# danieleschmidt/Graph-Hypernetwork-Forge

Measured on AMD Instinct MI355X. Metric: edges/s (HyperGNN forward), higher is better.
Workload: dtype f32; 1 GPU; synthetic uniform KG 1M nodes / 10M edges / 64 rel, hidden 128, L=3 (BASELINE config 3); nodes=1000000, edges=10000000, relations=64, hidden_dim=128, layers=3, text_dim=64, plan=cached (warm), launch=one C-ABI call per kernel, parallelism=single GPU

## Files before the change

### graph-hypernetwork-forge_amd/csrc/weightgen.hip

```cpp
#include "common.h"

namespace ghf {

constexpr int WG_MAX_WIDTH = 1024;
constexpr int WG_UNROLL = 8;
constexpr int WG_HU = 8;

struct HeadPtrs {
    const float* w[3][8];
    const float* b[3][8];
};
constexpr int WG_MAX_L = 8;
struct HeadPtrsL { HeadPtrs p[WG_MAX_L]; };

__global__ __launch_bounds__(256) void wg_hidden_kernel(const float* __restrict__ text_emb, HeadPtrsL PL,
                                                        int R, int T, int Hh, int num_hidden,
                                                        float* __restrict__ hidden_ws, float* __restrict__ acts,
                                                        const float* __restrict__ drop ) {
    __shared__ float buf[2][WG_MAX_WIDTH];
    const int r = blockIdx.x, head = blockIdx.y;
    const HeadPtrs& P = PL.p[blockIdx.z];
    if (hidden_ws) hidden_ws += (size_t)blockIdx.z * 3 * R * (num_hidden ? Hh : T);
    for (int k = threadIdx.x; k < T; k += blockDim.x) buf[0][k] = text_emb[(size_t)r * T + k];
    __syncthreads();
    int cur = 0, in_dim = T;
    const int lane = threadIdx.x & 63, wv = threadIdx.x >> 6, nw = blockDim.x >> 6;
    for (int li = 0; li < num_hidden; ++li) {
        const float* __restrict__ W = P.w[head][li];
        const float* __restrict__ B = P.b[head][li];
        for (int j0 = wv * WG_HU; j0 < Hh; j0 += nw * WG_HU) {
            float s[WG_HU];
#pragma unroll
            for (int u = 0; u < WG_HU; ++u) s[u] = 0.f;
            for (int k = lane; k < in_dim; k += 64) {
                const float xk = buf[cur][k];
#pragma unroll
                for (int u = 0; u < WG_HU; ++u)
                    if (j0 + u < Hh) s[u] = fmaf(xk, W[(size_t)(j0 + u) * in_dim + k], s[u]);
            }
#pragma unroll
            for (int u = 0; u < WG_HU; ++u) {
                const float t = wave_sum(s[u]);
                if (lane == 0 && j0 + u < Hh) {
                    const float a = fmaxf(t + B[j0 + u], 0.f);
                    buf[cur ^ 1][j0 + u] = drop ? a * drop[(((size_t)head * num_hidden + li) * R + r) * Hh + j0 + u] : a;
                }
            }
        }
        __syncthreads();
        cur ^= 1;
        in_dim = Hh;
        if (acts) {
            float* a = acts + (((size_t)head * num_hidden + li) * R + r) * Hh;
            for (int k = threadIdx.x; k < Hh; k += blockDim.x) a[k] = buf[cur][k];
        }
    }
    if (!hidden_ws) return;
    float* out = hidden_ws + ((size_t)head * R + r) * in_dim;
    for (int k = threadIdx.x; k < in_dim; k += blockDim.x) out[k] = buf[cur][k];
}

__device__ __forceinline__ size_t frag16_index(int r, int kk, int o, int d) {
    const int NT = d >> 4, NJ2 = d >> 3;
    return ((((size_t)r * NT + (o >> 4)) * NJ2 + (kk >> 4)) * 64 + (((kk & 15) >> 2) << 4) + (o & 15)) * 4 + (kk & 3);
}

__global__ __launch_bounds__(256) void wg_out_simple_kernel(const float* __restrict__ z ,
                                                            const float* __restrict__ W3, const float* __restrict__ b3,
                                                            const float* __restrict__ log_scale,
                                                            int R, int Hl, int n_out, int head, int d_in, int d_out,
                                                            int layout, size_t rstride, float* __restrict__ out) {
    const int lane = threadIdx.x & 63;
    const int n = blockIdx.x * 4 + (threadIdx.x >> 6);
    if (n >= n_out) return;
    const float scale = expf(log_scale[0]);
    const float bn = b3[n];
    for (int r0 = 0; r0 < R; r0 += WG_UNROLL) {
      float sv[WG_UNROLL];
#pragma unroll
      for (int u = 0; u < WG_UNROLL; ++u) sv[u] = 0.f;
      for (int k = lane; k < Hl; k += 64) {
          const float wk = W3[(size_t)n * Hl + k];
#pragma unroll
          for (int u = 0; u < WG_UNROLL; ++u)
              if (r0 + u < R) sv[u] = fmaf(z[(size_t)(r0 + u) * Hl + k], wk, sv[u]);
      }
#pragma unroll
      for (int u = 0; u < WG_UNROLL; ++u) {
        const int r = r0 + u;
        const float s = wave_sum(sv[u]);
        if (lane == 0 && r < R) {
            const float v = (s + bn) * scale;
            if (head == 2 || layout == GHF_WLAYOUT_NATURAL) {
                out[(size_t)r * rstride + n] = v;
            } else {
                const int i = n / d_out, o = n - i * d_out;
                out[frag16_index(r, head * d_in + i, o, d_out)] = v;
            }
        }
      }
    }
}

typedef float f32x4 __attribute__((ext_vector_type(4)));

template <int LAYOUT>
__global__ __launch_bounds__(256) void wg_out_mfma_kernel(const float* __restrict__ z ,
                                                          const float* __restrict__ W3, const float* __restrict__ b3,
                                                          const float* __restrict__ log_scale,
                                                          int R, int Hl, int n_out, int head, int d, size_t rstride,
                                                          float* __restrict__ out) {
    const int lane = threadIdx.x & 63, wv = threadIdx.x >> 6;
    const int q = lane >> 4, c16 = lane & 15;
    const int mt = blockIdx.x * 4 + wv;
    if (mt * 16 >= n_out) return;
    int n_a;
    int o = 0, it = 0;
    if (LAYOUT != GHF_WLAYOUT_NATURAL) {
        const int tiles_per_o = d >> 4;
        o = mt / tiles_per_o;
        it = mt - o * tiles_per_o;
        n_a = (16 * it + c16) * d + o;
    } else {
        n_a = 16 * mt + c16;
    }
    const bool a_ok = n_a < n_out;
    const float* __restrict__ arow = W3 + (size_t)(a_ok ? n_a : 0) * Hl + 4 * q;
    const float scale = expf(log_scale[0]);
    const int NJ = Hl >> 4;

    for (int r0 = 0; r0 < R; r0 += 16) {
        const int rc = r0 + c16;
        const bool b_ok = rc < R;
        const float* __restrict__ brow = z + (size_t)(b_ok ? rc : 0) * Hl + 4 * q;
        f32x4 acc = {0.f, 0.f, 0.f, 0.f};
        for (int j = 0; j < NJ; ++j) {
            f32x4 a = *(const f32x4*)(arow + 16 * j);
            f32x4 b = *(const f32x4*)(brow + 16 * j);
            if (!a_ok) a = (f32x4){0.f, 0.f, 0.f, 0.f};
            if (!b_ok) b = (f32x4){0.f, 0.f, 0.f, 0.f};
#pragma unroll
            for (int s = 0; s < 4; ++s) acc = __builtin_amdgcn_mfma_f32_16x16x4f32(a[s], b[s], acc, 0, 0, 0);
        }
        if (!b_ok) continue;
        if (LAYOUT == GHF_WLAYOUT_FRAG16) {
            f32x4 v;
#pragma unroll
            for (int s = 0; s < 4; ++s) {
                const int n = (16 * it + 4 * q + s) * d + o;
                v[s] = (acc[s] + b3[n]) * scale;
            }
            const int kk0 = head * d + 16 * it + 4 * q;
            *(f32x4*)(out + frag16_index(rc, kk0, o, d)) = v;
        } else {
#pragma unroll
            for (int s = 0; s < 4; ++s) {
                const int n = 16 * mt + 4 * q + s;
                if (n < n_out) out[(size_t)rc * rstride + n] = (acc[s] + b3[n]) * scale;
            }
        }
    }
}

struct OutHeads {
    const float* z[3];
    const float* W3[3];
    const float* b3[3];
    const float* log_scale[3];
    float* out[3];
    int n_out[3];
    size_t rstride[3];
};
struct OutHeadsL { OutHeads h[WG_MAX_L]; };
template <int NJT>
__global__ __launch_bounds__(256) void wg_out_mfma3_kernel(OutHeadsL HL, int R, int Hl) {
    const int head = blockIdx.y % 3;
    const OutHeads& H = HL.h[blockIdx.y / 3];
    const float* __restrict__ z = H.z[head];
    const float* __restrict__ W3 = H.W3[head];
    const float* __restrict__ b3 = H.b3[head];
    float* __restrict__ out = H.out[head];
    const int n_out = H.n_out[head];
    const size_t rstride = H.rstride[head];
    const int lane = threadIdx.x & 63, wv = threadIdx.x >> 6;
    const int q = lane >> 4, c16 = lane & 15;
    const int mt = blockIdx.x * 4 + wv;
    if (mt * 16 >= n_out) return;
    const int n_a = 16 * mt + c16;
    const bool a_ok = n_a < n_out;
    const float* __restrict__ arow = W3 + (size_t)(a_ok ? n_a : 0) * Hl + 4 * q;
    const float scale = expf(H.log_scale[head][0]);
    const int NJ = Hl >> 4;
    if constexpr (NJT > 0) {
        f32x4 a[NJT];
#pragma unroll
        for (int j = 0; j < NJT; ++j) {
            a[j] = *(const f32x4*)(arow + 16 * j);
            if (!a_ok) a[j] = (f32x4){0.f, 0.f, 0.f, 0.f};
        }
        for (int r0 = 0; r0 < R; r0 += 16) {
            const int rc = r0 + c16;
            const bool b_ok = rc < R;
            const float* __restrict__ brow = z + (size_t)(b_ok ? rc : 0) * Hl + 4 * q;
            f32x4 b[NJT];
#pragma unroll
            for (int j = 0; j < NJT; ++j) {
                b[j] = *(const f32x4*)(brow + 16 * j);
                if (!b_ok) b[j] = (f32x4){0.f, 0.f, 0.f, 0.f};
            }
            f32x4 acc = {0.f, 0.f, 0.f, 0.f};
#pragma unroll
            for (int j = 0; j < NJT; ++j)
#pragma unroll
                for (int s = 0; s < 4; ++s) acc = __builtin_amdgcn_mfma_f32_16x16x4f32(a[j][s], b[j][s], acc, 0, 0, 0);
            if (!b_ok) continue;
#pragma unroll
            for (int s = 0; s < 4; ++s) {
                const int n = 16 * mt + 4 * q + s;
                if (n < n_out) out[(size_t)rc * rstride + n] = (acc[s] + b3[n]) * scale;
            }
        }
        return;
    }
    for (int r0 = 0; r0 < R; r0 += 16) {
        const int rc = r0 + c16;
        const bool b_ok = rc < R;
        const float* __restrict__ brow = z + (size_t)(b_ok ? rc : 0) * Hl + 4 * q;
        f32x4 acc = {0.f, 0.f, 0.f, 0.f};
        for (int j = 0; j < NJ; ++j) {
            f32x4 a = *(const f32x4*)(arow + 16 * j);
            f32x4 b = *(const f32x4*)(brow + 16 * j);
            if (!a_ok) a = (f32x4){0.f, 0.f, 0.f, 0.f};
            if (!b_ok) b = (f32x4){0.f, 0.f, 0.f, 0.f};
#pragma unroll
            for (int s = 0; s < 4; ++s) acc = __builtin_amdgcn_mfma_f32_16x16x4f32(a[s], b[s], acc, 0, 0, 0);
        }
        if (!b_ok) continue;
#pragma unroll
        for (int s = 0; s < 4; ++s) {
            const int n = 16 * mt + 4 * q + s;
            if (n < n_out) out[(size_t)rc * rstride + n] = (acc[s] + b3[n]) * scale;
        }
    }
}

struct PackL { float* W[WG_MAX_L]; };
__global__ __launch_bounds__(1024) void wg_pack2h_kernel(PackL WL, int R, int d, int32_t* __restrict__ range_flag) {
    float* __restrict__ W = WL.W[blockIdx.y];
    float* __restrict__ scales = W + (size_t)R * 2 * d * d;
    extern __shared__ float wbuf[];
    __shared__ float red[16];
    __shared__ int cnt[2];
    __shared__ WeakRows weak_red[16];
    if (threadIdx.x < 2) cnt[threadIdx.x] = 0;
    const int r = blockIdx.x, tid = threadIdx.x, n = 2 * d * d;
    float* __restrict__ mine = W + (size_t)r * n;
    float mx = 0.f;
    for (int i = tid; i < n / 4; i += 1024) {
        const float4 v = ((const float4*)mine)[i];
        ((float4*)wbuf)[i] = v;
        mx = fmaxf(fmaxf(mx, fmaxf(fabsf(v.x), fabsf(v.y))), fmaxf(fabsf(v.z), fabsf(v.w)));
    }
    mx = wave_absmax(mx);
    if ((tid & 63) == 0) red[tid >> 6] = mx;
    __syncthreads();
    mx = 0.f;
    for (int i = 0; i < 16; ++i) mx = fmaxf(mx, red[i]);
    {
        WeakRows wr;
        wr.init();
        const int lane = tid & 63, wv = tid >> 6;
        for (int row = wv; row < 2 * d; row += 16) {
            float s = 0.f;
            for (int o = lane; o < d; o += 64) s += fabsf(wbuf[row * d + o]);
            wr.add(row >= d, wave_sum(s));
        }
        if (lane == 0) weak_red[wv] = wr;
    }
    const int sh = split2h_shift(mx);
    const float up = pow2f(sh);
    if (tid == 0) scales[r] = pow2f(-sh);
    const int NKS = d >> 4;
    _Float16* __restrict__ dst = (_Float16*)mine;
    for (int g = tid; g < n / 8; g += 1024) {
        const int slot = g & 63, fk = g >> 6;
        const int ks = fk % NKS, ct = fk / NKS;
        const int o = ct * 16 + (slot & 15), kk0 = ks * 32 + (slot >> 4) * 8;
        _Float16 hi[8], lo[8];
        int tiny = 0, nz = 0;
#pragma unroll
        for (int e = 0; e < 8; ++e) {
            const float xs = wbuf[(kk0 + e) * d + o] * up;
            split2h(xs, hi[e], lo[e]);
            tiny += range_tiny(xs);
            nz += xs != 0.f;
        }
        _Float16* p = dst + ((size_t)fk * 2 * 64 + slot) * 8;
#pragma unroll
        for (int e = 0; e < 8; ++e) { p[e] = hi[e]; p[512 + e] = lo[e]; }
        if (tiny) atomicAdd(&cnt[0], tiny);
        if (nz) atomicAdd(&cnt[1], nz);
    }
    __syncthreads();
    if (tid == 0) {
        range_raise(range_flag, GHF_RANGE_WEIGHTS, cnt[0], cnt[1]);
        WeakRows wr = weak_red[0];
        for (int i = 1; i < 16; ++i) wr.merge(weak_red[i]);
        range_raise_weak(range_flag, wr, d);
    }
}

int launch_weightgen_acts(const float* text_emb, const float* const* head_params, int R, int T, int Hh, int num_hidden,
                          float* acts, const float* hidden_drop, hipStream_t stream) {
    GHF_REQUIRE(R > 0 && T > 0 && num_hidden >= 0 && num_hidden <= 7, "weightgen_acts: bad shape");
    GHF_REQUIRE(T <= WG_MAX_WIDTH && Hh <= WG_MAX_WIDTH, "weightgen_acts: text_dim/hidden_dim > %d unsupported", WG_MAX_WIDTH);
    if (num_hidden == 0) return GHF_OK;
    HeadPtrsL PL;
    HeadPtrs& P = PL.p[0];
    const int nl = num_hidden + 1;
    for (int h = 0; h < 3; ++h)
        for (int l = 0; l < nl; ++l) {
            P.w[h][l] = head_params[(h * nl + l) * 2 + 0];
            P.b[h][l] = head_params[(h * nl + l) * 2 + 1];
        }
    wg_hidden_kernel<<<dim3(R, 3, 1), 256, 0, stream>>>(text_emb, PL, R, T, Hh, num_hidden, nullptr, acts, hidden_drop);
    GHF_LAUNCH_CHECK();
    return GHF_OK;
}

__global__ __launch_bounds__(256) void wg_combine_kernel(const float* __restrict__ top, const float* __restrict__ bottom,
                                                         int transpose, int d, float* __restrict__ out) {
    const int r = blockIdx.y;
    const int n = 2 * d * d;
    for (int idx = blockIdx.x * 256 + threadIdx.x; idx < n; idx += gridDim.x * 256) {
        const int kk = idx / d, o = idx - kk * d;
        const float* src = kk < d ? top : bottom;
        const int k = kk < d ? kk : kk - d;
        float v = 0.f;
        if (src) v = transpose ? src[((size_t)r * d + o) * d + k] : src[((size_t)r * d + k) * d + o];
        out[(size_t)r * n + idx] = v;
    }
}

__global__ __launch_bounds__(256) void wg_combine_frag16_kernel(const float* __restrict__ top, const float* __restrict__ bottom,
                                                                int transpose, int d, float* __restrict__ out) {
    const int r = blockIdx.y;
    const int n = 2 * d * d;
    for (int idx = blockIdx.x * 256 + threadIdx.x; idx < n; idx += gridDim.x * 256) {
        const int kk = idx / d, o = idx - kk * d;
        const float* src = kk < d ? top : bottom;
        const int k = kk < d ? kk : kk - d;
        float v = 0.f;
        if (src) v = transpose ? src[((size_t)r * d + o) * d + k] : src[((size_t)r * d + k) * d + o];
        out[frag16_index(r, kk, o, d)] = v;
    }
}

int launch_weights_pack(const float* top, const float* bottom, int transpose, int R, int d, int layout, float* out,
                        hipStream_t stream) {
    GHF_REQUIRE(R > 0 && d > 0 && out, "weights_pack: bad arguments");
    if (layout == GHF_WLAYOUT_FRAG16) {
        GHF_REQUIRE((d % 16) == 0, "weights_pack: FRAG16 needs d %% 16 == 0");
        wg_combine_frag16_kernel<<<dim3(32, (unsigned)R), 256, 0, stream>>>(top, bottom, transpose, d, out);
        GHF_LAUNCH_CHECK();
        return GHF_OK;
    }
    GHF_REQUIRE(layout == GHF_WLAYOUT_SPLIT2H, "weights_pack: layout %d is not packed from natural matrices here", layout);
    GHF_REQUIRE((d % 32) == 0 && (size_t)2 * d * d * 4 <= 128 * 1024, "weights_pack: SPLIT2H needs d %% 32 == 0, d <= 128");
    wg_combine_kernel<<<dim3(32, (unsigned)R), 256, 0, stream>>>(top, bottom, transpose, d, out);
    GHF_LAUNCH_CHECK();
    const size_t lds = (size_t)2 * d * d * 4;
    GHF_SET_MAX_LDS(wg_pack2h_kernel, lds);
    PackL WL;
    WL.W[0] = out;
    wg_pack2h_kernel<<<dim3(R, 1), 1024, lds, stream>>>(WL, R, d, range_flag_ptr());
    GHF_LAUNCH_CHECK();
    return GHF_OK;
}

int launch_weightgen_batched(int L, const float* text_emb, const float* const* head_params, const float* const* log_scales,
                             int R, int T, int Hh, int num_hidden, int d_in, int d_out, int layout,
                             float* hidden_ws, float* const* W_msg, float* const* W_self, float* const* bias,
                             const float* hidden_drop, hipStream_t stream, float* acts) {
    GHF_REQUIRE(L >= 1 && L <= WG_MAX_L, "weightgen: %d generators per call (1..%d)", L, WG_MAX_L);
    GHF_REQUIRE(R > 0 && T > 0 && d_in > 0 && d_out > 0, "weightgen: R, T, d_in, d_out must be positive");
    GHF_REQUIRE(num_hidden >= 0 && num_hidden <= 7, "weightgen: num_hidden=%d outside [0,7]", num_hidden);
    GHF_REQUIRE(num_hidden == 0 || Hh > 0, "weightgen: hidden_dim must be positive");
    GHF_REQUIRE(T <= WG_MAX_WIDTH && Hh <= WG_MAX_WIDTH, "weightgen: text_dim/hidden_dim > %d unsupported", WG_MAX_WIDTH);
    GHF_REQUIRE(layout == GHF_WLAYOUT_NATURAL || layout == GHF_WLAYOUT_FRAG16 || layout == GHF_WLAYOUT_SPLIT2H, "weightgen: bad layout %d", layout);
    GHF_REQUIRE((!hidden_drop && !acts) || L == 1, "weightgen: dropout masks / saved activations go with one generator per call");
    for (int g = 0; g < L; ++g) {
        GHF_REQUIRE(W_msg[g] && bias[g], "weightgen: null output pointer (generator %d)", g);
        if (layout == GHF_WLAYOUT_SPLIT2H)
            GHF_REQUIRE(d_in == d_out && (d_in % 32) == 0 && (size_t)2 * d_in * d_out * 4 <= 128 * 1024 && (!W_self || W_self[g] == nullptr),
                        "weightgen: SPLIT2H needs d_in == d_out, d %% 32 == 0, d <= 128 and W_self == NULL");
        if (layout == GHF_WLAYOUT_FRAG16)
            GHF_REQUIRE(d_in == d_out && (d_in % 16) == 0 && (!W_self || W_self[g] == nullptr),
                        "weightgen: FRAG16 needs d_in == d_out, d %% 16 == 0 and W_self == NULL");
        else if (layout == GHF_WLAYOUT_NATURAL)
            GHF_REQUIRE(W_self && W_self[g] != nullptr, "weightgen: NATURAL layout needs W_self");
    }
    HeadPtrsL PL;
    const int nl = num_hidden + 1;
    for (int g = 0; g < L; ++g)
        for (int h = 0; h < 3; ++h)
            for (int l = 0; l < nl; ++l) {
                PL.p[g].w[h][l] = head_params[((size_t)(g * 3 + h) * nl + l) * 2 + 0];
                PL.p[g].b[h][l] = head_params[((size_t)(g * 3 + h) * nl + l) * 2 + 1];
                GHF_REQUIRE(PL.p[g].w[h][l] && PL.p[g].b[h][l], "weightgen: null parameter pointer (generator %d head %d layer %d)", g, h, l);
            }
    wg_hidden_kernel<<<dim3(R, 3, L), 256, 0, stream>>>(text_emb, PL, R, T, Hh, num_hidden, hidden_ws, acts, hidden_drop);
    GHF_LAUNCH_CHECK();

    const int Hl = num_hidden ? Hh : T;
    const int n_mat = d_in * d_out;
    bool merged = (layout == GHF_WLAYOUT_NATURAL || layout == GHF_WLAYOUT_SPLIT2H) && (Hl % 16) == 0;
    OutHeadsL HL;
    if (merged)
        for (int g = 0; g < L; ++g) {
            OutHeads& H = HL.h[g];
            for (int head = 0; head < 3; ++head) {
                H.z[head] = hidden_ws + ((size_t)g * 3 + head) * R * Hl;
                H.W3[head] = PL.p[g].w[head][num_hidden];
                H.b3[head] = PL.p[g].b[head][num_hidden];
                H.log_scale[head] = log_scales[g * 3 + head];
                GHF_REQUIRE(H.log_scale[head], "weightgen: null log-scale pointer (generator %d head %d)", g, head);
                H.n_out[head] = head == 2 ? d_out : n_mat;
                H.rstride[head] = (layout == GHF_WLAYOUT_SPLIT2H && head != 2) ? (size_t)2 * n_mat : (size_t)H.n_out[head];
                H.out[head] = head == 2 ? bias[g] : (layout == GHF_WLAYOUT_SPLIT2H ? W_msg[g] + (size_t)head * n_mat : (head == 0 ? W_msg[g] : W_self[g]));
                merged = merged && ((((uintptr_t)H.W3[head] | (uintptr_t)H.z[head]) & 15) == 0);
            }
        }
    if (merged) {
        const int mtiles = (n_mat + 15) / 16;
        const dim3 og((mtiles + 3) / 4, 3 * L);
        switch (Hl) {
            case 32: wg_out_mfma3_kernel<2><<<og, 256, 0, stream>>>(HL, R, Hl); break;
            case 64: wg_out_mfma3_kernel<4><<<og, 256, 0, stream>>>(HL, R, Hl); break;
            case 128: wg_out_mfma3_kernel<8><<<og, 256, 0, stream>>>(HL, R, Hl); break;
            case 256: wg_out_mfma3_kernel<16><<<og, 256, 0, stream>>>(HL, R, Hl); break;
            default: wg_out_mfma3_kernel<0><<<og, 256, 0, stream>>>(HL, R, Hl); break;
        }
        GHF_LAUNCH_CHECK();
    } else {
        for (int g = 0; g < L; ++g)
            for (int head = 0; head < 3; ++head) {
                const float* z = hidden_ws + ((size_t)g * 3 + head) * R * Hl;
                const float* W3 = PL.p[g].w[head][num_hidden];
                const float* b3 = PL.p[g].b[head][num_hidden];
                const float* ls = log_scales[g * 3 + head];
                GHF_REQUIRE(ls, "weightgen: null log-scale pointer (generator %d head %d)", g, head);
                const int n_out = head == 2 ? d_out : n_mat;
                const bool nat = layout == GHF_WLAYOUT_NATURAL || layout == GHF_WLAYOUT_SPLIT2H;
                const size_t rstride = (layout == GHF_WLAYOUT_SPLIT2H && head != 2) ? (size_t)2 * n_mat : (size_t)n_out;
                float* out = head == 2 ? bias[g] : (layout == GHF_WLAYOUT_SPLIT2H ? W_msg[g] + (size_t)head * n_mat
                                                    : (layout != GHF_WLAYOUT_NATURAL ? W_msg[g] : (head == 0 ? W_msg[g] : W_self[g])));
                const int klayout = nat ? GHF_WLAYOUT_NATURAL : layout;
                const bool mfma_ok = (Hl % 16) == 0 && ((((uintptr_t)W3 | (uintptr_t)z) & 15) == 0);
                if (mfma_ok && layout == GHF_WLAYOUT_FRAG16 && head != 2) {
                    const int mtiles = n_mat / 16;
                    wg_out_mfma_kernel<GHF_WLAYOUT_FRAG16><<<(mtiles + 3) / 4, 256, 0, stream>>>(z, W3, b3, ls, R, Hl, n_out, head, d_out, rstride, out);
                } else if (mfma_ok) {
                    const int mtiles = (n_out + 15) / 16;
                    wg_out_mfma_kernel<GHF_WLAYOUT_NATURAL><<<(mtiles + 3) / 4, 256, 0, stream>>>(z, W3, b3, ls, R, Hl, n_out, head, d_out, rstride, out);
                } else {
                    wg_out_simple_kernel<<<(n_out + 3) / 4, 256, 0, stream>>>(z, W3, b3, ls, R, Hl, n_out, head, d_in, d_out, klayout, rstride, out);
                }
                GHF_LAUNCH_CHECK();
            }
    }
    if (layout == GHF_WLAYOUT_SPLIT2H) {
        const size_t lds = (size_t)2 * n_mat * 4;
        PackL WL;
        for (int g = 0; g < L; ++g) WL.W[g] = W_msg[g];
        GHF_SET_MAX_LDS(wg_pack2h_kernel, lds);
        wg_pack2h_kernel<<<dim3(R, L), 1024, lds, stream>>>(WL, R, d_out, range_flag_ptr());
        GHF_LAUNCH_CHECK();
    }
    return GHF_OK;
}

int launch_weightgen(const float* text_emb, const float* const* head_params, const float* const* log_scales,
                     int R, int T, int Hh, int num_hidden, int d_in, int d_out, int layout,
                     float* hidden_ws, float* W_msg, float* W_self, float* bias, const float* hidden_drop, hipStream_t stream,
                     float* acts) {
    float* wm[1] = {W_msg};
    float* wsf[1] = {W_self};
    float* bs[1] = {bias};
    return launch_weightgen_batched(1, text_emb, head_params, log_scales, R, T, Hh, num_hidden, d_in, d_out, layout, hidden_ws,
                                    wm, wsf, bs, hidden_drop, stream, acts);
}

}
```

Before: 1.051 billion edges/s.

## Batch four relations per block in weight-generator hidden MLP kernel

Adds a hidden-layer kernel in which each 1024-thread block handles four relations at once, keeping their activations in dynamic LDS. Each weight row load is reused across all four relations instead of being reloaded per relation. The 32 wave reductions are gathered into lanes with writelane, so lanes can write outputs in parallel. The cost is more registers per thread and fewer blocks, which for R=64 means only 16x3xL blocks and may reduce GPU occupancy.

Measured after the change: 1.064 billion edges/s (median of 6 runs). +1.2%, better.

```diff
diff --git a/graph-hypernetwork-forge_amd/csrc/weightgen.hip b/graph-hypernetwork-forge_amd/csrc/weightgen.hip
--- a/graph-hypernetwork-forge_amd/csrc/weightgen.hip
+++ b/graph-hypernetwork-forge_amd/csrc/weightgen.hip
@@ -58,6 +58,80 @@
     if (!hidden_ws) return;
     float* out = hidden_ws + ((size_t)head * R + r) * in_dim;
     for (int k = threadIdx.x; k < in_dim; k += blockDim.x) out[k] = buf[cur][k];
+}
+
+constexpr int WG_RB = 4;
+constexpr int WG_HT = 1024;
+__global__ __launch_bounds__(WG_HT) void wg_hidden_rb_kernel(const float* __restrict__ text_emb, HeadPtrsL PL,
+                                                             int R, int T, int Hh, int num_hidden, int width,
+                                                             float* __restrict__ hidden_ws, float* __restrict__ acts,
+                                                             const float* __restrict__ drop ) {
+    extern __shared__ float hbuf[];
+    const int r0 = blockIdx.x * WG_RB, head = blockIdx.y;
+    const int nr = R - r0 < WG_RB ? R - r0 : WG_RB;
+    const HeadPtrs& P = PL.p[blockIdx.z];
+    if (hidden_ws) hidden_ws += (size_t)blockIdx.z * 3 * R * (num_hidden ? Hh : T);
+    float* cur = hbuf;
+    float* nxt = hbuf + (size_t)WG_RB * width;
+    for (int i = threadIdx.x; i < WG_RB * T; i += blockDim.x) {
+        const int rr = i / T, k = i - rr * T;
+        cur[rr * width + k] = rr < nr ? text_emb[(size_t)(r0 + rr) * T + k] : 0.f;
+    }
+    __syncthreads();
+    int in_dim = T;
+    const int lane = threadIdx.x & 63, wv = threadIdx.x >> 6, nw = blockDim.x >> 6;
+    const int lr = lane / WG_HU, lu = lane % WG_HU;
+    for (int li = 0; li < num_hidden; ++li) {
+        const float* __restrict__ W = P.w[head][li];
+        const float* __restrict__ B = P.b[head][li];
+        for (int j0 = wv * WG_HU; j0 < Hh; j0 += nw * WG_HU) {
+            float s[WG_RB][WG_HU];
+#pragma unroll
+            for (int rr = 0; rr < WG_RB; ++rr)
+#pragma unroll
+                for (int u = 0; u < WG_HU; ++u) s[rr][u] = 0.f;
+            for (int k = lane; k < in_dim; k += 64) {
+                float w[WG_HU];
+#pragma unroll
+                for (int u = 0; u < WG_HU; ++u) {
+                    const int j = j0 + u < Hh ? j0 + u : Hh - 1;
+                    w[u] = W[(size_t)j * in_dim + k];
+                }
+#pragma unroll
+                for (int rr = 0; rr < WG_RB; ++rr) {
+                    const float xk = cur[rr * width + k];
+#pragma unroll
+                    for (int u = 0; u < WG_HU; ++u) s[rr][u] = fmaf(xk, w[u], s[rr][u]);
+                }
+            }
+            float t = 0.f;
+#pragma unroll
+            for (int rr = 0; rr < WG_RB; ++rr)
+#pragma unroll
+                for (int u = 0; u < WG_HU; ++u) {
+                    const float tu = wave_sum(s[rr][u]);
+                    asm("v_writelane_b32 %0, %1, %2" : "+v"(t) : "s"(tu), "n"(rr * WG_HU + u));
+                }
+            const int j = j0 + lu;
+            if (lane < WG_RB * WG_HU && lr < nr && j < Hh) {
+                const float a = fmaxf(t + B[j], 0.f);
+                nxt[lr * width + j] = drop ? a * drop[(((size_t)head * num_hidden + li) * R + r0 + lr) * Hh + j] : a;
+            }
+        }
+        __syncthreads();
+        float* sw = cur; cur = nxt; nxt = sw;
+        in_dim = Hh;
+        if (acts)
+            for (int i = threadIdx.x; i < nr * Hh; i += blockDim.x) {
+                const int rr = i / Hh, k = i - rr * Hh;
+                acts[(((size_t)head * num_hidden + li) * R + r0 + rr) * Hh + k] = cur[rr * width + k];
+            }
+    }
+    if (!hidden_ws) return;
+    for (int i = threadIdx.x; i < nr * in_dim; i += blockDim.x) {
+        const int rr = i / in_dim, k = i - rr * in_dim;
+        hidden_ws[((size_t)head * R + r0 + rr) * in_dim + k] = cur[rr * width + k];
+    }
 }
 
 __device__ __forceinline__ size_t frag16_index(int r, int kk, int o, int d) {
@@ -409,7 +483,12 @@
                 PL.p[g].b[h][l] = head_params[((size_t)(g * 3 + h) * nl + l) * 2 + 1];
                 GHF_REQUIRE(PL.p[g].w[h][l] && PL.p[g].b[h][l], "weightgen: null parameter pointer (generator %d head %d layer %d)", g, h, l);
             }
-    wg_hidden_kernel<<<dim3(R, 3, L), 256, 0, stream>>>(text_emb, PL, R, T, Hh, num_hidden, hidden_ws, acts, hidden_drop);
+    {
+        const int width = T > Hh ? T : Hh;
+        const size_t lds = (size_t)2 * WG_RB * width * sizeof(float);
+        wg_hidden_rb_kernel<<<dim3((R + WG_RB - 1) / WG_RB, 3, L), WG_HT, lds, stream>>>(text_emb, PL, R, T, Hh, num_hidden, width,
+                                                                                    hidden_ws, acts, hidden_drop);
+    }
     GHF_LAUNCH_CHECK();
 
     const int Hl = num_hidden ? Hh : T;
```
